# Shadylukin/Neumann

Measured on AMD Instinct MI355X. Metric: queries/sec, brute-force SIMILAR TOP-K (recall@K = 1.0 vs CPU oracle), higher is better.
Workload: dtype f32

## Files before the change

### neumann_amd/csrc/nmn_api.hip

```cpp
#include <algorithm>
#include <atomic>
#include <chrono>
#include <thread>
#include <cmath>
#include <cstdio>
#include <cstdlib>
#include <cstring>
#include <mutex>
#include <new>
#include <string>
#include <unordered_map>
#include <vector>

#include "nmn_index.h"

using namespace nmn;

namespace nmn {
float synth_value_host(uint64_t seed, uint64_t row, uint32_t col);
}

static thread_local std::string g_last_error;

static nmn_status fail_hip(hipError_t e, const char* what) {
// ... 950 lines not shown
        if (qmasks_host && !use_mfma) {
            const bool mark = w->timed && qa == 0 && !nested;
            if (mark && (st = hist_mark(0)) != NMN_OK) return st;
            for (uint32_t i = 0; i < nqc; i++) {
                st = search_enqueue(idx, w, queries_dev + (size_t)(qa + i) * idx->dim, 1, k, metric, qmasks_host[qa + i],
                                    out_rows + (size_t)(qa + i) * k, out_scores + (size_t)(qa + i) * k, out_counts + qa + i,
                                    stream, nullptr, nullptr, short_chain, true);
                if (st != NMN_OK) return st;
            }
            if (mark && (st = hist_mark(1)) != NMN_OK) return st;
            continue;
        }
        w->last_elem_bytes = use_i8 ? 1u : use_half ? 2u : 4u;
        static const bool two_planes = env_set("NMN_I8_TWO_PLANES");
        const bool pipelined = idx->sweep_seq != 0 && idx->sweep_stream != stream;
        const bool one_plane = use_i8 && use_mfma && !two_planes && metric == NMN_METRIC_COSINE && k <= 128u && (nqc > 64u || !pipelined) &&
                               scan_mfma_i8_one_plane_supported((int)metric) && idx->q8_calls >= idx->one_plane_off_until;
        if (one_plane) idx->one_plane_recent = true;
        const bool f32_retry = (use_half || use_i8) && !use_mfma && n_rows >= (1u << 18) && !short_chain;
        static const bool no_run_bound = env_set("NMN_NO_RUN_BOUND");
        static const bool wgs_pinned = getenv("NMN_MFMA_WGS") != nullptr;
        const bool run_bound = use_mfma && !no_run_bound && !no_sample() && !mask_dev && !qmasks_dev && k <= 256u && nqc <= 64u && !wgs_pinned &&
                               idx->ld <= 1536u &&
                               n_tiles >= 1024u * kSampleStep && n_tiles / kSampleStep >= 4u * k;
        const uint32_t run_S = run_bound ? k : 0u;
        HIP_TRY(launch_qprep(queries_dev + (size_t)qa * idx->dim, nqc, idx->dim, idx->ld, (int)metric,
                             idx->max_norm_bits, w->qpad, w->qinfo, w->qstate,
                             use_i8 ? (1 | 2 | 4 | (use_mfma ? (one_plane ? 16 : 0) : 8)) : ((use_mfma ? 1 : 0) | ((use_half || mfma_f32) ? 2 : 0)), stream,
                             use_i8 ? idx->q8_err_bits : (use_half || (mfma_f32 && idx->half && idx->half_rows >= n_rows)) ? idx->half_err_bits : nullptr,
                             use_i8 ? w->qi8 : nullptr,
                             (use_i8 && !use_mfma) ? idx->q8_l2_hint : nullptr, f32_retry ? w->qinfo_f32 : nullptr,
                             run_bound ? w->run_slots : nullptr, run_S, run_bound ? w->run_bound : nullptr));
        if (n_rows > 0) {
            ScanParams sp{};
            sp.corpus = idx->corpus;
            sp.corpus_half = use_half ? idx->half : nullptr;
            sp.corpus_i8 = use_i8 ? idx->q8 : nullptr;
            sp.i8_one_plane = one_plane ? 1u : 0u;
            sp.i8_scale = idx->q8_scale;
            sp.i8_vv = idx->q8_vv;
            sp.i8_cos = idx->q8_cos;
            sp.qi8 = w->qi8;
            sp.norms = idx->norms;
            sp.inv_norms = idx->inv_norms;
            sp.qpad = w->qpad;
            sp.qinfo = w->qinfo;
            sp.mask = mask_dev;
// ... 11 lines not shown
            static const uint32_t wave_target = [] {
                const char* e = getenv("NMN_SCAN_WAVES");
                long v = e ? atol(e) : (long)kMaxScanWaves;
                return (uint32_t)std::min<long>(std::max<long>(v, 256), (long)kMaxScanWaves);
            }();
            sp.tiles_per_wave = std::max<uint32_t>(1, (n_tiles + wave_target - 1) / wave_target);
            static const bool waves_pinned = getenv("NMN_SCAN_WAVES") != nullptr;
            static const uint32_t small_waves = [] {
                const char* e = getenv("NMN_SCAN_WAVES_SMALL");
                const long v = e ? atol(e) : 768;
                return v <= 0 ? 0u : (uint32_t)std::min<long>(std::max<long>(v, 256), (long)kMaxScanWaves);
            }();
            {
                const uint64_t sweep_bytes = (uint64_t)n_rows * idx->ld * w->last_elem_bytes;
                if (!waves_pinned && small_waves && !use_mfma && !mask_dev && sweep_bytes >= (128ull << 20) && sweep_bytes < (2ull << 30))
                    sp.tiles_per_wave = std::max<uint32_t>(1, (n_tiles + small_waves - 1) / small_waves);
            }
            static const uint32_t mfma_wgs = [] {
                const char* e = getenv("NMN_MFMA_WGS");
                long v = e ? atol(e) : 1024;
                return (uint32_t)std::min<long>(std::max<long>(v, 64), (long)kMaxScanWaves);
            }();
            if (use_mfma) sp.tiles_per_wave = std::max<uint32_t>(1, (n_tiles + mfma_wgs - 1) / mfma_wgs);
            auto launch_batch_sweep = [&](const ScanParams& x) -> hipError_t { return launch_scan_mfma(x, stream); };
            static const bool no_ring = getenv("NMN_NO_RING") != nullptr;
            const bool use_ring = !no_ring && !use_mfma && !use_i8 && !use_half && nqc == 1 && !mask_dev && !qmasks_dev && n_tiles >= 4096u &&
                                  metric != NMN_METRIC_SPARSE_COSINE_F64 && scan_ring_supported(idx->ld, idx->dim, (int)metric);
            static const uint32_t ring_wgs = [] {
                const char* e = getenv("NMN_RING_WGS");
                long v = e ? atol(e) : (long)kMaxScanWaves;
                return (uint32_t)std::min<long>(std::max<long>(v, 64), (long)kMaxScanWaves);
            }();
            if (use_ring) sp.tiles_per_wave = std::max<uint32_t>(1, (n_tiles + ring_wgs - 1) / ring_wgs);
            ring_set_grid(sp, use_ring ? w->ring_ctr : nullptr);
            sp.metric = (int)metric;
            sp.strided = (!use_mfma && mask_dev) ? 1u : 0u;
            static const bool no_walk = getenv("NMN_NO_WALK") != nullptr;
            sp.walk = (sp.strided && !no_walk) ? 1u : 0u;
            sp.tile_step = 1;
            sp.skip_key = nullptr;
            static const uint32_t sample_step = [] {
                const char* e = getenv("NMN_SAMPLE_STEP");
                const long v = e ? atol(e) : 0;
                return (v == 64 || v == 128 || v == 256) ? (uint32_t)v : kSampleStep;
            }();
            static const bool sample_behind = getenv("NMN_SAMPLE_AHEAD_OF_CHAIN") == nullptr;
// ... 13 lines not shown
                ss.n_tiles = n_sample;
                ss.tiles_per_wave = std::max<uint32_t>(1, (n_sample + 255) / 256);
                ss.tmax = w->tsample;
                ss.tmax_stride = w->n_sample_cap;
                static const bool reread_env = getenv("NMN_SAMPLE_REREAD") != nullptr;
                const bool reread = reread_env || use_i8;
                if (!reread) {
                    ss.tmax_main = w->tmax;
                    ss.tmax_main_stride = w->tmax_stride;
                }
                HIP_TRY(launch_batch_sweep(ss));
                HIP_TRY(launch_sample_bound(w->tsample, w->n_sample_cap, n_sample, w->qinfo, nqc, k, w->skip_key, stream));
                sp.skip_key = w->skip_key;
                sp.skip_sampled = reread ? 0u : sample_step;
                return NMN_OK;
            };
            if (sample && !sample_behind) {
                st = sampling_pass();
                if (st != NMN_OK) return st;
            }
            static const bool no_chain = getenv("NMN_NO_SWEEP_CHAIN") != nullptr;
            const bool chain = !no_chain && (uint64_t)n_rows * idx->ld * w->last_elem_bytes >= (2ull << 30);
            if (sp.ring_wgs) HIP_TRY(hipMemsetAsync(w->wmax, 0, (size_t)((n_tiles + sp.tiles_per_wave - 1) / sp.tiles_per_wave) * sizeof(uint32_t), stream));
            if (chain && idx->sweep_seq && idx->sweep_stream != stream)
                HIP_TRY(hipStreamWaitEvent(stream, idx->sweep_ev[(idx->sweep_seq - 1) & 3u], 0));
            if (w->timed && qa == 0 && !nested) {
                hipEvent_t& h = w->hist[2 * (w->hist_head % Workspace::kTimingHistory)];
                if (!h) HIP_TRY(hipEventCreate(&h));
                HIP_TRY(hipEventRecord(h, stream));
            }
            if (sample && sample_behind) {
                st = sampling_pass();
                if (st != NMN_OK) return st;
            }
            static const bool no_refine = getenv("NMN_NO_REFINE") != nullptr;
            const uint32_t mfma_blocks = use_mfma ? (n_tiles + sp.tiles_per_wave - 1) / sp.tiles_per_wave : 0;
            static const uint32_t n_cu = [] {
                int dev = 0, n = 256;
                if (hipGetDevice(&dev) != hipSuccess || hipDeviceGetAttribute(&n, hipDeviceAttributeMultiprocessorCount, dev) != hipSuccess || n <= 0) n = 256;
                return (uint32_t)n;
            }();
            const uint32_t first_blocks = mfma_blocks >= 3u * n_cu ? (n_cu & ~7u) : 0u;
            static const uint32_t refine_min_nq = [] {
                const char* e = getenv("NMN_REFINE_MIN_NQ");
                return e ? (uint32_t)atol(e) : 65u;
            }();
// ... 1152 lines not shown
```

### neumann_amd/csrc/nmn_internal.h

```cpp
#pragma once
#include <hip/hip_runtime.h>
#include <stdint.h>

#include "../../include/neumann_gpu.h"

namespace nmn {

constexpr int kMetricNegL2 = 16;
constexpr int kMetricNegL2Sq = 17;

constexpr uint32_t kTileRows = 64;
constexpr uint32_t kDefaultCandCap = 4096;
constexpr uint32_t kMaxScanWaves = 4096;
constexpr uint32_t kKeyMasked = 0u;
constexpr uint32_t kKeyNaN = 1u;
constexpr uint32_t kScoreSentinelBits = 0xFFFFFFFFu;

struct QInfo {
    float qmag;
    float margin_abs;
    float margin_rel;
    float pad;
    float qscale;
    float qq8;
// ... 99 lines not shown
    uint64_t n_rows;
    uint32_t nql;
    uint32_t tile_step;
    uint32_t fold_ny;
    const uint32_t* skip_key;
    uint32_t* tmax_main;
    uint64_t tmax_main_stride;
    uint32_t skip_sampled;
    uint32_t ld;
    uint32_t n_tiles;
    uint32_t nq;
    uint32_t tiles_per_wave;
    uint32_t strided;
    uint32_t walk;
    uint32_t bx_base, bx_count;
    uint32_t* run_slots;
    uint32_t* run_bound;
    uint32_t run_S;
    uint32_t i8_one_plane;
    uint32_t ring_wgs;
    uint32_t ring_tail;
    uint32_t ring_grid;
    uint32_t* ring_ctr;
    uint32_t run_dbg;
    int metric;
};
hipError_t launch_scan(const ScanParams& p, hipStream_t s);
bool scan_ring_supported(uint32_t ld, uint32_t dim, int metric);
hipError_t launch_scan_ring(const ScanParams& p, hipStream_t s);
hipError_t launch_half_rows(const float* corpus, float* half, uint32_t ld, uint64_t row0, uint64_t n, const float* norms,
                            float* row_err2_scratch, uint32_t* err_bits, hipStream_t s);
bool scan_half_supported(uint32_t ld, int metric);
bool scan_i8_supported(uint32_t ld, uint32_t dim, int metric);
hipError_t launch_scan_i8(const ScanParams& p, hipStream_t s);
hipError_t launch_q8_rows(const float* corpus, int8_t* q8, float* scale, float* vv, float* cosf, uint32_t ld, uint64_t row0, uint64_t n, const float* norms,
                          float* row_err2_scratch, uint32_t* err_bits, hipStream_t s);
bool ingest_supported(uint32_t ld, uint32_t dim);
bool exact_rows_supported(uint32_t ld, uint32_t dim, int metric);
hipError_t launch_exact_rows(const float* corpus, const float* norms, uint32_t ld, uint64_t n_rows, const float* qpad, const QInfo* qinfo,
                             const QState* qstate, int flagged, const uint64_t* mask, const uint64_t* const* qmasks, uint32_t* scores,
                             uint32_t nql, uint32_t nq, int metric, hipStream_t s);
hipError_t launch_ingest(const float* corpus, uint32_t ld, uint64_t row0, uint64_t n, float* norms, float* inv_norms,
                         uint32_t* max_norm_bits, float* half, uint32_t* err_bits, hipStream_t s);
bool ingest_q8_supported(uint32_t ld, uint32_t dim);
hipError_t launch_ingest_q8(const float* corpus, uint32_t ld, uint64_t row0, uint64_t n, float* norms, float* inv_norms, uint32_t* max_norm_bits,
                            int8_t* q8, float* scale, float* vv, float* cosf, uint32_t* err_bits, hipStream_t s);
hipError_t launch_read_probe(const float* corpus, uint64_t n_rows, uint32_t ld, float* sink, hipStream_t s);
hipError_t launch_ring_probe(const float* corpus, uint64_t n_rows, uint32_t ld, uint32_t tiles_per_wg, uint32_t* ctr, hipStream_t s);
void ring_set_grid(ScanParams& p, uint32_t* ctr);
bool scan_mfma_supported(uint32_t ld, uint32_t dim, int metric);
hipError_t launch_scan_mfma(const ScanParams& p, hipStream_t s);
hipError_t launch_scan_mfma_f32(const ScanParams& p, hipStream_t s);
bool scan_mfma_i8_supported(uint32_t ld, uint32_t dim, int metric);
bool scan_mfma_i8_one_plane_supported(int metric);
hipError_t launch_scan_mfma_i8_one(const ScanParams& p, hipStream_t s);

struct SelectParams {
    const uint32_t* scores;
    const uint32_t* tmax;
    const uint32_t* wmax;
    uint64_t tmax_stride;
    uint64_t wmax_stride;
    uint32_t n_waves;
    uint32_t tiles_per_wave;
    uint32_t strided;
    const QInfo* qinfo;
    QState* qstate;
    uint32_t* cand_rows;
    uint64_t n_rows;
    uint32_t nql;
    uint32_t n_tiles;
    uint32_t nq;
// ... 177 lines not shown
```

### neumann_amd/csrc/nmn_scan_mfma.hip

```cpp
#include "nmn_scan_mfma_kernel.h"

namespace nmn {

template <int KC, int KS, int QG, int METRIC, int WAVES = 4>
static hipError_t launch_kc(const ScanParams& p, hipStream_t s) {
    return (p.mask || p.qmasks) ? launch_one_mfma<KC, KS, QG, METRIC, true, WAVES>(p, s)
                                : launch_one_mfma<KC, KS, QG, METRIC, false, WAVES>(p, s);
}

template <int METRIC>
static hipError_t launch_metric(const ScanParams& p, hipStream_t s) {
    static const bool waves8 = [] {
        const char* e = getenv("NMN_MFMA_WAVES");
        return e ? atoi(e) == 8 : false;
    }();
    if (waves8) {
        if (p.nq > 64) {
            switch (p.ld / kStageK) {
                case 6: return launch_kc<3, 2, 8, METRIC, 8>(p, s);
                default: break;
            }
        } else {
            switch (p.ld / kStageK) {
                case 6: return launch_kc<3, 2, 4, METRIC, 8>(p, s);
// ... 72 lines not shown
        case 5: return launch_kc_i8<5, 1, METRIC>(p, s);
        case 6: return launch_kc_i8<3, 2, METRIC>(p, s);
        case 8: return launch_kc_i8<4, 2, METRIC, 2>(p, s);
        case 12: return launch_kc_i8<6, 2, METRIC, 2>(p, s);
        default: return hipErrorInvalidValue;
    }
}
bool scan_mfma_i8_supported(uint32_t ld, uint32_t dim, int metric) {
    if (!(metric == NMN_METRIC_COSINE || metric == NMN_METRIC_DOT_PRODUCT || metric == NMN_METRIC_EUCLIDEAN || metric == kMetricNegL2))
        return false;
    if (ld == 3072u && (metric == NMN_METRIC_EUCLIDEAN || metric == kMetricNegL2)) return false;
    return dim <= ld && ld % 256u == 0 && ld >= 256u && (ld <= 1536u || ld == 2048u || ld == 3072u);
}

bool scan_mfma_supported(uint32_t ld, uint32_t dim, int metric) {
    if (!(metric == NMN_METRIC_COSINE || metric == NMN_METRIC_DOT_PRODUCT || metric == NMN_METRIC_EUCLIDEAN ||
          metric == kMetricNegL2) ||
        dim > ld || ld % kStageK != 0)
        return false;
    const uint32_t kc = ld / kStageK;
    return (kc >= 1 && kc <= 6) || kc == 8 || kc == 10 || kc == 12 || kc == 16 || kc == 24 || kc == 32;
}

hipError_t launch_scan_mfma(const ScanParams& p, hipStream_t s) {
    if (!p.corpus_i8 && !p.corpus_half) return launch_scan_mfma_f32(p, s);
    if (p.corpus_i8 && p.i8_one_plane) return launch_scan_mfma_i8_one(p, s);
    if (p.corpus_i8) {
        switch (p.metric) {
            case NMN_METRIC_COSINE: return launch_metric_i8<NMN_METRIC_COSINE>(p, s);
            case NMN_METRIC_EUCLIDEAN: return launch_metric_i8<NMN_METRIC_EUCLIDEAN>(p, s);
            case kMetricNegL2: return launch_metric_i8<kMetricNegL2>(p, s);
            default: return launch_metric_i8<NMN_METRIC_DOT_PRODUCT>(p, s);
        }
    }
    switch (p.metric) {
        case NMN_METRIC_COSINE: return launch_metric<NMN_METRIC_COSINE>(p, s);
        case NMN_METRIC_EUCLIDEAN: return launch_metric<NMN_METRIC_EUCLIDEAN>(p, s);
        case kMetricNegL2: return launch_metric<kMetricNegL2>(p, s);
        default: return launch_metric<NMN_METRIC_DOT_PRODUCT>(p, s);
    }
}

}
```

### neumann_amd/csrc/nmn_scan_mfma_kernel.h

```cpp
#pragma once
#include <algorithm>
#include <cstdlib>
#include <type_traits>

#include "nmn_internal.h"

namespace nmn {

typedef float f4 __attribute__((ext_vector_type(4)));
typedef short s8 __attribute__((ext_vector_type(8)));
typedef uint32_t u4 __attribute__((ext_vector_type(4)));

#ifndef NMN_MFMA_BATCH
#define NMN_MFMA_BATCH 8
#endif
constexpr int kStageK = 128;
#ifndef NMN_MFMA_RING_KB
#define NMN_MFMA_RING_KB 128
#endif
#ifndef NMN_MFMA_OCC
#define NMN_MFMA_OCC 1
#endif
#ifdef NMN_MFMA_NO_FENCES
#define NMN_MFMA_FENCE() do { } while (0)
#else
#define NMN_MFMA_FENCE() __builtin_amdgcn_sched_barrier(0)
#endif
constexpr int kRingBytes = NMN_MFMA_RING_KB * 1024;

typedef float f2 __attribute__((ext_vector_type(2)));
typedef __bf16 bf2 __attribute__((ext_vector_type(2)));

__device__ __forceinline__ uint32_t cvt_pk_bf16(float lo, float hi) {
    const f2 v = {lo, hi};
    return __builtin_bit_cast(uint32_t, __builtin_convertvector(v, bf2));
}

__device__ __forceinline__ s8 to_bf16x8(const f4& a, const f4& b) {
    u4 h;
    h[0] = cvt_pk_bf16(a.x, a.y);
    h[1] = cvt_pk_bf16(a.z, a.w);
    h[2] = cvt_pk_bf16(b.x, b.y);
    h[3] = cvt_pk_bf16(b.z, b.w);
    return __builtin_bit_cast(s8, h);
}

constexpr int kNormSlots = 16;

template <int AUX, int PIECES>
__device__ __forceinline__ void stage_dma(const char* stage_base, const uint32_t (&loff)[PIECES], float* buf,
                                          uint32_t wave) {
#pragma unroll
    for (int pp = 0; pp < PIECES; pp++) {
        const char* src = stage_base + loff[pp];
        __builtin_amdgcn_global_load_lds((const __attribute__((address_space(1))) void*)src,
                                         (__attribute__((address_space(3))) void*)(buf + (wave * PIECES + (uint32_t)pp) * 256u),
                                         16, 0, AUX);
    }
}

template <int AUX, int PIECES>
__device__ __forceinline__ void stage_dma_piece(const char* stage_base, const uint32_t (&loff)[PIECES], float* buf, uint32_t wave,
                                                int pp) {
    __builtin_amdgcn_global_load_lds((const __attribute__((address_space(1))) void*)(stage_base + loff[pp]),
                                     (__attribute__((address_space(3))) void*)(buf + (wave * PIECES + (uint32_t)pp) * 256u), 16, 0, AUX);
}

__device__ __forceinline__ void norms_dma(const float* __restrict__ norms, uint64_t tile, float* nbuf, uint32_t lane) {
// ... 32 lines not shown
    const float d2 = __builtin_fmaxf(__builtin_fmaf(-2.0f, dot, qq8 + vv), 0.0f);
    const float d = __builtin_amdgcn_sqrtf(d2);
    return NEG ? -d : __builtin_amdgcn_rcpf(1.0f + d);
}

template <int KS, int QG, int WAVES, bool I8>
__host__ __device__ constexpr uint32_t kRunLdsBase() {
    return (uint32_t)(kRingBytes + kNormSlots * 64 * 4 + (QG * 2 == WAVES ? QG * 64 * 4 * 16 : 0) +
                      WAVES * (QG * 2 == WAVES ? 1 : QG / WAVES) * 16 * 16 +
#ifdef NMN_MFMA_PACK
                      (I8 ? kNormSlots * 64 * 4 + WAVES * (16 * 64 + 16) * 4 : 0));
#else
                      (I8 ? kNormSlots * 64 * 4 : 0));
#endif
}
constexpr int kRunVals = 1024;
template <int QG>
__host__ __device__ constexpr uint32_t kRunLdsRing() { return (uint32_t)(kNormSlots * QG * 16 * 4); }
template <int QG, int WAVES>
__host__ __device__ constexpr uint32_t kRunLdsBytes() {
    return kRunLdsRing<QG>() + (uint32_t)(QG * 16 * (int)sizeof(QInfo) + WAVES * kRunVals * 4);
}

template <int KC, int KS, int QG, int METRIC, bool MASKED, int AUX, int WAVES, bool I8 = false, bool F32 = false, bool ONE = false>
__global__ void __launch_bounds__(WAVES * 64, NMN_MFMA_OCC) scan_mfma_kernel(ScanParams p) {
    static_assert(!(I8 && F32), "one streamed matrix");
    static_assert(!ONE || I8, "one query plane: the 8-bit form only");
    constexpr int kStageElems = 128 * KS;
    constexpr int kStageBytes = kTileRows * kStageElems * 2;
    constexpr int kRowPitch = kStageElems / 2;
    constexpr int kRing = kRingBytes / kStageBytes;
    constexpr int kPieces = 16 * KS / WAVES;
    constexpr uint32_t LR = 16 * KS;
    constexpr bool kL2 = METRIC == NMN_METRIC_EUCLIDEAN || METRIC == kMetricNegL2;
    constexpr bool kNeedNorms = I8 || METRIC == NMN_METRIC_COSINE || kL2;
    constexpr bool kScaled = METRIC == NMN_METRIC_COSINE || (I8 && METRIC == NMN_METRIC_DOT_PRODUCT);
    extern __shared__ __attribute__((aligned(16))) float lds[];
    float* nrm = lds + kRingBytes / 4;
    float* const nrm2 = nrm + kNormSlots * 64 + (QG * 2 == WAVES ? QG * 64 * 16 : 0) + WAVES * (QG * 2 == WAVES ? 1 : QG / WAVES) * 16 * 4;
#ifdef NMN_MFMA_PACK
    constexpr bool kPack = I8;
#else
    constexpr bool kPack = false;
#endif
    float* const pack_lds = nrm2 + kNormSlots * 64;
    constexpr uint32_t kQ = (uint32_t)QG * 16u;
    uint32_t* const bnd = reinterpret_cast<uint32_t*>(lds) + (kRunLdsBase<KS, QG, WAVES, I8>() >> 2);
    QInfo* const qmrg = reinterpret_cast<QInfo*>(bnd + kNormSlots * kQ);
    uint32_t* const slotb = reinterpret_cast<uint32_t*>(qmrg + kQ);
    const uint32_t run_S = p.run_S;
    const uint32_t lane = threadIdx.x & 63u;
    const uint32_t wave = __builtin_amdgcn_readfirstlane(threadIdx.x >> 6);
    const uint32_t g = lane >> 4, n = lane & 15u;
    const uint32_t ld = p.ld;
    const uint32_t row_bytes = I8 ? ld : F32 ? ld * 4u : ld * 2u;
    uint32_t bx = blockIdx.x, by = blockIdx.y;
    if (p.fold_ny > 1) {
        const uint32_t span = 8u * p.fold_ny, grp_ = blockIdx.x / span, r_ = blockIdx.x % span;
        by = r_ / 8u;
        bx = grp_ * 8u + (r_ % 8u);
    }
    if (p.bx_count && bx >= p.bx_count) return;
    bx += p.bx_base;
    const uint32_t q0 = by * (uint32_t)(QG * 16);
    constexpr bool kHalfK = QG * 2 == WAVES;
    static_assert(kHalfK || QG % WAVES == 0, "query groups: one (or more) per wave, or one per wave PAIR");
    const uint32_t grp = kHalfK ? (wave % (uint32_t)QG) : wave;
    const uint32_t kh = kHalfK ? (wave / (uint32_t)QG) : 0u;

    constexpr int kStageSteps = F32 ? 2 * KS : 4 * KS;
    constexpr int kSteps = kHalfK ? kStageSteps / 2 : kStageSteps;
    static_assert(kSteps >= 1, "K-halves need two k-steps per stage");
    constexpr int kBK = KC * kSteps;
    constexpr int kBG = kHalfK ? 1 : QG / WAVES;
    s8 bhi[kBK][kBG];
    s8 blo[(I8 && !ONE) ? kBK : 1][kBG];
#pragma unroll
    for (int qg = 0; qg < kBG; qg++) {
        const uint32_t qq = q0 + ((uint32_t)qg * (uint32_t)WAVES + grp) * 16u + n;
        const bool ok = qq < p.nq;
        const float* qv = p.qpad + (size_t)(ok ? qq : q0) * ld;
        if constexpr (I8) {
            const char* qb = reinterpret_cast<const char*>(p.qi8) + (size_t)(ok ? qq : q0) * 2u * ld;
#pragma unroll
            for (int kc = 0; kc < kBK; kc++) {
                const uint32_t k0b = ((uint32_t)(kc / kSteps) * (4u * KS) + kh * (uint32_t)kSteps + (uint32_t)(kc % kSteps)) * 64u + g * 16u;
// ... 36 lines not shown
        skip_h[h] = (q_ok_h[h] && p.skip_key) ? p.skip_key[qn_h[h]] : kKeyNaN;
        wmax_h[h] = kKeyMasked;
    }

    if (run_S) {
        for (uint32_t i = threadIdx.x; i < kQ; i += (uint32_t)WAVES * 64u)
            qmrg[i] = p.qinfo[min(q0 + i, p.nq - 1u)];
        __syncthreads();
    }
#ifndef NMN_RUN_PICK
#define NMN_RUN_PICK 4
#endif
    constexpr uint32_t kPick = NMN_RUN_PICK;
    auto bound_dma = [&](uint32_t rel) __attribute__((always_inline)) {
        if (rel % kPick) return;
#pragma unroll
        for (uint32_t h = 0; h < kQ; h += 64u)
            __builtin_amdgcn_global_load_lds((const __attribute__((address_space(1))) void*)(p.run_bound + q0 + h + lane),
                                             (__attribute__((address_space(3))) void*)(bnd + ((rel / kPick) % kNormSlots) * kQ + h), 4, 0, 16);
    };
    uint32_t pend_q = 0xFFFFFFFFu;
    const uint32_t tstep = p.tile_step;
    const bool sampling = tstep > 1;
    const uint32_t t0 = bx * p.tiles_per_wave;
    if (t0 >= p.n_tiles) return;
    const uint32_t t1 = min(t0 + p.tiles_per_wave, p.n_tiles);
    const uint32_t S = sampling ? 0u : p.skip_sampled;
    auto walked_below = [&](uint32_t t) -> uint32_t { return S ? t - (t + S - 1u) / S : t; };
    auto tile_of = [&](uint32_t j) -> uint32_t { return S ? j + j / (S - 1u) + 1u : j; };
    const uint32_t j0 = walked_below(t0), j1 = walked_below(t1);
    const uint32_t n_stage = (j1 - j0) * KC;

    uint32_t loff[kPieces];
#pragma unroll
    for (int pp = 0; pp < kPieces; pp++) {
        const uint32_t r = (64u / LR) * (wave * kPieces + (uint32_t)pp) + lane / LR;
        loff[pp] = r * row_bytes + (((lane % LR) ^ (r & 15u)) * 16u);
    }
    const char* const mirror = I8 ? reinterpret_cast<const char*>(p.corpus_i8)
                                  : F32 ? reinterpret_cast<const char*>(p.corpus) : reinterpret_cast<const char*>(p.corpus_half);
    const float* const norm_src = I8 ? (METRIC == NMN_METRIC_COSINE ? p.i8_cos : p.i8_scale)
                                     : (METRIC == NMN_METRIC_COSINE ? p.inv_norms : p.norms);
    auto stage_src = [&](uint32_t tile_, uint32_t kc_) -> const char* {
        return mirror + (uint64_t)tile_ * tstep * kTileRows * row_bytes + (uint64_t)kc_ * (kStageElems * 2u);
    };

#pragma unroll
    for (uint32_t s0 = 0; s0 < kRing; s0++) {
        if (s0 < n_stage) {
            if (run_S && !(p.run_dbg & 8u) && wave == 0 && s0 % KC == 0) bound_dma(s0 / KC);
            if (kNeedNorms && wave == 0 && s0 % KC == 0)
            {
                norms_dma(norm_src, (uint64_t)tile_of(j0 + s0 / KC) * tstep, nrm + ((s0 / KC) % kNormSlots) * 64u, lane);
                if constexpr (I8 && kL2) norms_dma(p.i8_vv, (uint64_t)tile_of(j0 + s0 / KC) * tstep, nrm2 + ((s0 / KC) % kNormSlots) * 64u, lane);
            }
            if (s0 < kRing - 1)
                stage_dma<AUX, kPieces>(stage_src(tile_of(j0 + s0 / KC), s0 % KC), loff, lds + (s0 % kRing) * (kStageBytes / 4), wave);
        } else if (s0 < kRing - 1) {
            const uint32_t zero[kPieces] = {};
            stage_dma<AUX, kPieces>(mirror, zero, lds + (s0 % kRing) * (kStageBytes / 4), wave);
        }
    }

    uint32_t off[kSteps];
#pragma unroll
    for (int ks = 0; ks < kSteps; ks++)
        off[ks] = F32 ? n * kRowPitch + ((((kh * (uint32_t)kSteps + (uint32_t)ks) * 8u + g * 2u) ^ n) * 4u)
                      : n * kRowPitch + ((((kh * (uint32_t)kSteps + (uint32_t)ks) * 4u + g) ^ n) * 4u);
// ... 35 lines not shown
            if (q_ok && g == 0) p.tmax[(uint64_t)qn * p.tmax_stride + ftile] = tkey;
#else
            {
                const uint32_t slot = ftile & 3u;
                uint32_t* mine = tk_pend + (((uint32_t)wave * (uint32_t)kHalves + (uint32_t)H) * 16u + n) * 4u;
                if (g == 0) mine[slot] = tkey;
                if (slot == 3u || flast) {
                    const uint32_t g0 = ftile & ~3u, first = max((S && g0 % S == 0u) ? g0 + 1u : g0, t0);
                    if (q_ok && g == 0) {
                        uint32_t* dst = p.tmax + (uint64_t)qn * p.tmax_stride + g0;
                        const u4 v = *reinterpret_cast<const u4*>(mine);
                        if (first == g0 && slot == 3u && (p.tmax_stride & 3ull) == 0ull) {
                            *reinterpret_cast<u4*>(dst) = v;
                        } else {
                            if (first <= g0 + 0u) dst[0] = v[0];
                            if (first <= g0 + 1u && slot >= 1u) dst[1] = v[1];
                            if (first <= g0 + 2u && slot >= 2u) dst[2] = v[2];
                            if (first <= g0 + 3u && slot >= 3u) dst[3] = v[3];
                        }
                    }
                }
            }
#endif
            if (run_S && !(p.run_dbg & 2u) && q_ok && g == 0 && tkey > wmax_h[H] && !sampling) p.run_slots[(size_t)qn * (uint32_t)kRunVals + bx] = tkey;
            wmax_h[H] = max(wmax_h[H], tkey);
            const bool finish_sampled = sampling && p.tmax_main != nullptr;
            if (finish_sampled && q_ok && g == 0) p.tmax_main[(uint64_t)qn * p.tmax_main_stride + rtile] = tkey;
#ifdef NMN_MFMA_NO_SCORE_WRITES
            return false;
#else
            const bool wr_ = q_ok && (!sampling || finish_sampled) && tkey != kKeyMasked && tkey >= skip;
            return wr_;
#endif
        };
        constexpr bool kLazy = METRIC == NMN_METRIC_COSINE || METRIC == NMN_METRIC_DOT_PRODUCT;
        auto l2_of = [&](float acc_v, float vn_v, float vv_v) __attribute__((always_inline)) -> float {
            if constexpr (I8) return l2_score_i8<METRIC == kMetricNegL2>(qq, vv_v, acc_v * (inv_q * vn_v));
            else return l2_score<METRIC == kMetricNegL2>(qq, vn_v, acc_v);
        };
        if (mword == ~0ull) {
            float m = -__builtin_inff();
            u4 bits[4];
#pragma unroll
            for (int rb = 0; rb < 4; rb++) {
                f4 sc = fin[rb];
                if constexpr (kScaled) {
                    sc = sc * npre[rb];
// ... 36 lines not shown
#pragma unroll
                        for (int rb = 0; rb < 4; rb++) *reinterpret_cast<u4*>(stage + rank * 64u + (uint32_t)rb * 16u + g * 4u) = words(rb);
                        if (g == 0) qsel[rank] = qn;
                    }
                    asm volatile("" ::: "memory");
                    const uint32_t nw = (uint32_t)__builtin_popcount(qm);
                    for (uint32_t b = 0; b < nw; b += 4u) {
                        const uint32_t slot = b + (lane >> 4), piece = lane & 15u;
                        if (slot < nw) {
                            const u4 v = *reinterpret_cast<const u4*>(stage + slot * 64u + piece * 4u);
                            *reinterpret_cast<u4*>(p.scores + score_at(r0 + piece * 4u, qsel[slot], p.nql)) = v;
                        }
                    }
                    asm volatile("" ::: "memory");
                }
            } else if (wr) {
#pragma unroll
                for (int rb = 0; rb < 4; rb++)
                    *reinterpret_cast<u4*>(p.scores + score_at(r0 + (uint32_t)rb * 16u + g * 4u, qn, p.nql)) = words(rb);
            }
        } else {
            uint32_t tkey = kKeyMasked;
            u4 bits[4];
#pragma unroll
            for (int rb = 0; rb < 4; rb++) {
                const uint32_t rr = (uint32_t)rb * 16u + g * 4u;
                f4 vn = {1.f, 1.f, 1.f, 1.f}, vv = {0.f, 0.f, 0.f, 0.f};
                if constexpr (kNeedNorms) vn = npre[rb];
                if constexpr (I8 && kL2) vv = *reinterpret_cast<const f4*>(nslot2 + rr);
#pragma unroll
                for (int e = 0; e < 4; e++) {
                    const bool valid = ((mword >> (rr + (uint32_t)e)) & 1ull) != 0;
                    float sc = fin[rb][e];
                    if constexpr (kScaled) sc = (sc * vn[e]) * inv_q;
                    if constexpr (kL2) sc = l2_of(sc, vn[e], vv[e]);
                    bits[rb][e] = valid ? f2u(sc) : kScoreSentinelBits;
                    if (valid) tkey = max(tkey, score_to_key(sc));
                }
            }
            if (publish(tkey)) {
#pragma unroll
                for (int rb = 0; rb < 4; rb++)
                    *reinterpret_cast<u4*>(p.scores + score_at(r0 + (uint32_t)rb * 16u + g * 4u, qn, p.nql)) = bits[rb];
            }
        }
    };
    auto finish_tile = [&](const f4 (&facc)[4][kAccGroups], uint32_t ftile, uint32_t frel, bool flast, const f4 (&npre)[4],
                           const uint32_t (&skp)[kHalves]) __attribute__((always_inline)) {
#ifdef NMN_MFMA_NO_EPILOGUE
// ... 16 lines not shown
        const uint32_t tile = tile_of(j);
        f4 acc[4][kAccGroups];
        f4 npre[4] = {{1.f, 1.f, 1.f, 1.f}, {1.f, 1.f, 1.f, 1.f}, {1.f, 1.f, 1.f, 1.f}, {1.f, 1.f, 1.f, 1.f}};
        uint32_t skp[kHalves];
#pragma unroll
        for (int h = 0; h < kHalves; h++) skp[h] = kKeyNaN;
        v4i ach[I8 ? 4 : 1][kAccGroups], acl[I8 ? 4 : 1][kAccGroups];
#pragma unroll
        for (int rb = 0; rb < 4; rb++)
#pragma unroll
            for (int qg = 0; qg < kAccGroups; qg++) {
                acc[rb][qg] = (f4){0.f, 0.f, 0.f, 0.f};
                if constexpr (I8) {
                    ach[rb][qg] = (v4i){0, 0, 0, 0};
                    acl[rb][qg] = (v4i){0, 0, 0, 0};
                }
            }
#pragma unroll
        for (int kc = 0; kc < KC; kc++, sidx++) {
            const float* buf = lds + (sidx % kRing) * (kStageBytes / 4);
            wait_vm_imm<(kRing - 2) * kPieces>();
            __builtin_amdgcn_s_barrier();
            asm volatile("" ::: "memory");
            const uint32_t ns = sidx + (kRing - 1);
            const bool issue = ns < n_stage;
            const uint32_t nt = tile_of(j0 + ns / KC), nkc = ns % KC;
            const char* const nsrc = issue ? stage_src(nt, nkc) : mirror;
            const uint32_t lmask = issue ? 0xFFFFFFFFu : 0u;
            float* const nbuf = lds + (ns % kRing) * (kStageBytes / 4);
            constexpr int kKsPerBatch = F32 ? 1 : (kBK * kBG * (I8 ? 8 : 4) >= (I8 ? 192 : 256)) ? 1 : 2;
            static_assert(kSteps % kKsPerBatch == 0, "batches tile the stage");
            constexpr int kNB = kSteps / kKsPerBatch;
            s8 a[F32 ? 1 : kSteps][4];
            u4 raw[F32 ? kSteps : 1][4][2];
            auto read_batch = [&](int b) __attribute__((always_inline)) {
#pragma unroll
                for (int ks = b * kKsPerBatch; ks < (b + 1) * kKsPerBatch; ks++)
#pragma unroll
                    for (int rb = 0; rb < 4; rb++) {
                        if constexpr (F32) {
                            const uint32_t o0 = off[ks], o1 = off[ks] ^ 4u;
                            raw[ks][rb][0] = *reinterpret_cast<const u4*>(buf + rb * 16 * kRowPitch + o0);
                            raw[ks][rb][1] = *reinterpret_cast<const u4*>(buf + rb * 16 * kRowPitch + o1);
                        } else {
                            a[ks][rb] = __builtin_bit_cast(s8, *reinterpret_cast<const u4*>(buf + rb * 16 * kRowPitch + off[ks]));
                        }
                    }
            };
// ... 90 lines not shown
                for (int rb = 0; rb < 4; rb++)
                    *reinterpret_cast<f4*>(xch + ((grp * 64u + lane) * 4u + (uint32_t)rb) * 4u) = acc[rb][0];
            }
            asm volatile("s_waitcnt lgkmcnt(0)" ::: "memory");
            __builtin_amdgcn_s_barrier();
            asm volatile("" ::: "memory");
            if (kh == 0) {
#pragma unroll
                for (int rb = 0; rb < 4; rb++)
                    acc[rb][0] += *reinterpret_cast<const f4*>(xch + ((grp * 64u + lane) * 4u + (uint32_t)rb) * 4u);
            }
            asm volatile("s_waitcnt lgkmcnt(0)" ::: "memory");
            finish_tile(acc, tile, j - j0, j + 1u == j1, npre, skp);
        } else {
            finish_tile(acc, tile, j - j0, j + 1u == j1, npre, skp);
        }
        if (run_S && !(p.run_dbg & 4u)) {
#ifndef NMN_RUN_REFRESH
#define NMN_RUN_REFRESH 64
#endif
            constexpr uint32_t kRefresh = NMN_RUN_REFRESH;
            constexpr uint32_t kDelay = (uint32_t)((kRing - 2 + KC - 1) / KC);
            static_assert(kDelay >= 1 && kDelay < kRefresh, "refresh timing");
            const uint32_t rel = j - j0, phase = bx % kRefresh;
            if ((rel % kRefresh) == (phase + kDelay) % kRefresh && pend_q != 0xFFFFFFFFu) {
                wait_vm_imm<(kRing - 2) * kPieces>();
                uint32_t v[kRunVals / 64];
#pragma unroll
                for (int i = 0; i < kRunVals / 256; i++) {
                    const u4 x = *reinterpret_cast<const u4*>(slotb + wave * (uint32_t)kRunVals + (uint32_t)i * 256u + lane * 4u);
                    v[4 * i + 0] = x[0]; v[4 * i + 1] = x[1]; v[4 * i + 2] = x[2]; v[4 * i + 3] = x[3];
                }
                uint32_t pre = 0;
                for (int bit = 31; bit >= 10; bit--) {
                    const uint32_t c = pre | (1u << bit);
                    uint32_t cnt = 0;
#pragma unroll
                    for (int i = 0; i < kRunVals / 64; i++) cnt += (uint32_t)__builtin_popcountll(__ballot(v[i] >= c));
                    if (cnt >= run_S) pre = c;
                }
                if (pre > kKeyNaN && lane == 0) atomicMax(p.run_bound + pend_q, margin_key(pre, qmrg[pend_q - q0]));
            }
            if ((rel % kRefresh) == phase) {
                const uint32_t turn = ((rel / kRefresh) + bx) % (16u * (uint32_t)kBG);
                const uint32_t qq = q0 + ((turn / 16u) * (uint32_t)WAVES + grp) * 16u + (turn % 16u);
                pend_q = (kh == 0 && qq < p.nq) ? qq : 0xFFFFFFFFu;
                if (pend_q != 0xFFFFFFFFu) {
#pragma unroll
                    for (int i = 0; i < kRunVals / 256; i++)
                        __builtin_amdgcn_global_load_lds((const __attribute__((address_space(1))) void*)(p.run_slots + (size_t)pend_q * (uint32_t)kRunVals + (uint32_t)i * 256u + lane * 4u),
                                                         (__attribute__((address_space(3))) void*)(slotb + wave * (uint32_t)kRunVals + (uint32_t)i * 256u), 16, 0, 16);
                }
            }
        }
    }
    wait_vm_imm<0>();
    if (sampling) return;
#pragma unroll
    for (int h = 0; h < kHalves; h++)
        if (q_ok_h[h] && g == 0) {
            if (S)
                for (uint32_t ts = ((t0 + S - 1u) / S) * S; ts < t1; ts += S)
                    wmax_h[h] = max(wmax_h[h], p.tmax[(uint64_t)qn_h[h] * p.tmax_stride + ts]);
            p.wmax[(size_t)qn_h[h] * p.wmax_stride + bx] = wmax_h[h];
        }
}

template <int KC, int KS, int QG, int METRIC, bool MASKED, int WAVES, bool I8 = false, bool F32 = false, bool ONE = false>
static hipError_t launch_one_mfma(const ScanParams& p, hipStream_t s) {
    const uint32_t blocks_all = (p.n_tiles + p.tiles_per_wave - 1) / p.tiles_per_wave;
    if (p.bx_base >= blocks_all) return hipSuccess;
    const uint32_t blocks = p.bx_count ? std::min(p.bx_count, blocks_all - p.bx_base) : blocks_all - p.bx_base;
    const uint32_t ny = (p.nq + QG * 16 - 1) / (QG * 16);
    ScanParams pf = p;
    pf.bx_count = blocks;
    dim3 grid(blocks, ny);
    static const bool no_fold = getenv("NMN_MFMA_NO_FOLD") != nullptr;
    if (ny > 1 && !no_fold) {
        pf.fold_ny = ny;
        grid = dim3(((blocks + 7u) / 8u) * 8u * ny, 1);
    }
    const size_t lds = (size_t)kRunLdsBase<KS, QG, WAVES, I8>() + (p.run_S ? (size_t)kRunLdsBytes<QG, WAVES>() : (size_t)kRunLdsRing<QG>());
    if (lds > 160u * 1024u) return hipErrorInvalidValue;
    if (p.skip_sampled && (p.skip_sampled < 4u || (p.skip_sampled & 3u))) return hipErrorInvalidValue;
    if (p.run_S && (p.run_S > 256u || blocks_all > (uint32_t)kRunVals || p.tile_step > 1u || (p.skip_sampled && !(p.run_dbg & 1u)))) return hipErrorInvalidValue;
#ifndef NMN_MFMA_AUX
#define NMN_MFMA_AUX 2
#endif
    auto kern = scan_mfma_kernel<KC, KS, QG, METRIC, MASKED, NMN_MFMA_AUX, WAVES, I8, F32, ONE>;
    hipError_t e = hipFuncSetAttribute(reinterpret_cast<const void*>(kern), hipFuncAttributeMaxDynamicSharedMemorySize,
                                       (int)lds);
    if (e != hipSuccess) return e;
    hipLaunchKernelGGL(kern, grid, dim3(WAVES * 64), lds, s, pf);
    return hipGetLastError();
}

}
```

Baseline: 225.7.

## Add persistent one-launch MFMA sweep with atomic-ticket work stealing over split tile chunks

Under the run-bound path, the MFMA scan kernel now launches one workgroup per CU. Each workgroup pulls chunk tickets from an atomic counter, and each 1024-way tile group is divided into several parts, with finer parts for the tail groups. Partial per-group maxima are merged with atomicMax into run_slots and wmax, which are cleared beforehand with a memset. The goal is to remove tail imbalance and wave quantization across CUs. The cost is atomics, extra barriers per chunk, a memset, and a counter that the last workgroup must reset.

New measurement: 225.2, median of 2. No clear change (-0.2%).

```diff
diff --git a/neumann_amd/csrc/nmn_api.hip b/neumann_amd/csrc/nmn_api.hip
--- a/neumann_amd/csrc/nmn_api.hip
+++ b/neumann_amd/csrc/nmn_api.hip
@@ -996,7 +996,8 @@
         static const bool wgs_pinned = getenv("NMN_MFMA_WGS") != nullptr;
         const bool run_bound = use_mfma && !no_run_bound && !no_sample() && !mask_dev && !qmasks_dev && k <= 256u && nqc <= 64u && !wgs_pinned &&
                                idx->ld <= 1536u &&
-                               n_tiles >= 1024u * kSampleStep && n_tiles / kSampleStep >= 4u * k;
+                               n_tiles >= 1024u * kSampleStep && n_tiles / kSampleStep >= 4u * k &&
+                               scan_mfma_run_bound_fits(idx->ld, use_i8 ? 1u : use_half ? 2u : 4u, nqc);
         const uint32_t run_S = run_bound ? k : 0u;
         HIP_TRY(launch_qprep(queries_dev + (size_t)qa * idx->dim, nqc, idx->dim, idx->ld, (int)metric,
                              idx->max_norm_bits, w->qpad, w->qinfo, w->qstate,
@@ -1054,6 +1055,7 @@
                 return (uint32_t)std::min<long>(std::max<long>(v, 64), (long)kMaxScanWaves);
             }();
             if (use_mfma) sp.tiles_per_wave = std::max<uint32_t>(1, (n_tiles + mfma_wgs - 1) / mfma_wgs);
+            if (use_mfma) mfma_set_grid(sp, run_bound ? w->ring_ctr : nullptr);
             auto launch_batch_sweep = [&](const ScanParams& x) -> hipError_t { return launch_scan_mfma(x, stream); };
             static const bool no_ring = getenv("NMN_NO_RING") != nullptr;
             const bool use_ring = !no_ring && !use_mfma && !use_i8 && !use_half && nqc == 1 && !mask_dev && !qmasks_dev && n_tiles >= 4096u &&
@@ -1113,6 +1115,8 @@
             static const bool no_chain = getenv("NMN_NO_SWEEP_CHAIN") != nullptr;
             const bool chain = !no_chain && (uint64_t)n_rows * idx->ld * w->last_elem_bytes >= (2ull << 30);
             if (sp.ring_wgs) HIP_TRY(hipMemsetAsync(w->wmax, 0, (size_t)((n_tiles + sp.tiles_per_wave - 1) / sp.tiles_per_wave) * sizeof(uint32_t), stream));
+            if (use_mfma && sp.even_chunks)
+                HIP_TRY(hipMemset2DAsync(w->wmax, (size_t)kMaxScanWaves * sizeof(uint32_t), 0, (size_t)((n_tiles + sp.tiles_per_wave - 1) / sp.tiles_per_wave) * sizeof(uint32_t), nqc, stream));
             if (chain && idx->sweep_seq && idx->sweep_stream != stream)
                 HIP_TRY(hipStreamWaitEvent(stream, idx->sweep_ev[(idx->sweep_seq - 1) & 3u], 0));
             if (w->timed && qa == 0 && !nested) {
diff --git a/neumann_amd/csrc/nmn_internal.h b/neumann_amd/csrc/nmn_internal.h
--- a/neumann_amd/csrc/nmn_internal.h
+++ b/neumann_amd/csrc/nmn_internal.h
@@ -145,6 +145,8 @@
     uint32_t ring_tail;
     uint32_t ring_grid;
     uint32_t* ring_ctr;
+    uint32_t even_chunks, even_main_groups, even_main_parts, even_tail_parts, even_align, even_grid;
+    uint32_t* even_ctr;
     uint32_t run_dbg;
     int metric;
 };
@@ -171,6 +173,8 @@
 hipError_t launch_read_probe(const float* corpus, uint64_t n_rows, uint32_t ld, float* sink, hipStream_t s);
 hipError_t launch_ring_probe(const float* corpus, uint64_t n_rows, uint32_t ld, uint32_t tiles_per_wg, uint32_t* ctr, hipStream_t s);
 void ring_set_grid(ScanParams& p, uint32_t* ctr);
+void mfma_set_grid(ScanParams& p, uint32_t* ctr);
+bool scan_mfma_run_bound_fits(uint32_t ld, uint32_t elem_bytes, uint32_t nq);
 bool scan_mfma_supported(uint32_t ld, uint32_t dim, int metric);
 hipError_t launch_scan_mfma(const ScanParams& p, hipStream_t s);
 hipError_t launch_scan_mfma_f32(const ScanParams& p, hipStream_t s);
diff --git a/neumann_amd/csrc/nmn_scan_mfma.hip b/neumann_amd/csrc/nmn_scan_mfma.hip
--- a/neumann_amd/csrc/nmn_scan_mfma.hip
+++ b/neumann_amd/csrc/nmn_scan_mfma.hip
@@ -118,6 +118,31 @@
     return (kc >= 1 && kc <= 6) || kc == 8 || kc == 10 || kc == 12 || kc == 16 || kc == 24 || kc == 32;
 }
 
+bool scan_mfma_run_bound_fits(uint32_t ld, uint32_t elem_bytes, uint32_t nq) {
+    if (nq > 64u || ld > 1536u) return false;
+    const uint32_t lds = (elem_bytes == 1u ? kRunLdsBase<1, 4, 4, true>() : kRunLdsBase<1, 4, 4, false>()) + kRunLdsBytes<4, 4>() + kEvenLdsBytes;
+    return lds <= 160u * 1024u;
+}
+
+void mfma_set_grid(ScanParams& p, uint32_t* ctr) {
+    struct Knobs {
+        bool on;
+        uint32_t main, tail, align, cus;
+    };
+    static const Knobs k = []() -> Knobs {
+        int dev = 0, n = 256;
+        if (hipGetDevice(&dev) != hipSuccess || hipDeviceGetAttribute(&n, hipDeviceAttributeMultiprocessorCount, dev) != hipSuccess || n <= 0) n = 256;
+        auto knob = [](const char* name, long def, long lo, long hi) {
+            const char* e = getenv(name);
+            return (uint32_t)std::min<long>(std::max<long>(e ? atol(e) : def, lo), hi);
+        };
+        return {getenv("NMN_NO_MFMA_EVEN") == nullptr, knob("NMN_MFMA_MAIN", 6, 1, 1024), knob("NMN_MFMA_TAIL", 8, 0, 4096), knob("NMN_MFMA_ALIGN", 4, 1, 64),
+                (uint32_t)n};
+    }();
+    p.even_chunks = 0;
+    if (ctr && k.on) mfma_even_split(p, k.main, k.tail, k.align, k.cus, ctr);
+}
+
 hipError_t launch_scan_mfma(const ScanParams& p, hipStream_t s) {
     if (!p.corpus_i8 && !p.corpus_half) return launch_scan_mfma_f32(p, s);
     if (p.corpus_i8 && p.i8_one_plane) return launch_scan_mfma_i8_one(p, s);
diff --git a/neumann_amd/csrc/nmn_scan_mfma_kernel.h b/neumann_amd/csrc/nmn_scan_mfma_kernel.h
--- a/neumann_amd/csrc/nmn_scan_mfma_kernel.h
+++ b/neumann_amd/csrc/nmn_scan_mfma_kernel.h
@@ -44,6 +44,13 @@
     h[3] = cvt_pk_bf16(b.z, b.w);
     return __builtin_bit_cast(s8, h);
 }
+
+#ifdef NMN_MFMA_WG_CLOCK
+__device__ unsigned long long* nmn_mfma_clk;
+#define NMN_MFMA_CLK(i, v) do { if (threadIdx.x == 0) nmn_mfma_clk[(uint64_t)blockIdx.x * 5u + (i)] = (v); } while (0)
+#else
+#define NMN_MFMA_CLK(i, v) do { } while (0)
+#endif
 
 constexpr int kNormSlots = 16;
 
@@ -122,7 +129,9 @@
     return kRunLdsRing<QG>() + (uint32_t)(QG * 16 * (int)sizeof(QInfo) + WAVES * kRunVals * 4);
 }
 
-template <int KC, int KS, int QG, int METRIC, bool MASKED, int AUX, int WAVES, bool I8 = false, bool F32 = false, bool ONE = false>
+constexpr uint32_t kEvenLdsBytes = 16;
+
+template <int KC, int KS, int QG, int METRIC, bool MASKED, int AUX, int WAVES, bool I8 = false, bool F32 = false, bool ONE = false, bool EVEN = false>
 __global__ void __launch_bounds__(WAVES * 64, NMN_MFMA_OCC) scan_mfma_kernel(ScanParams p) {
     static_assert(!(I8 && F32), "one streamed matrix");
     static_assert(!ONE || I8, "one query plane: the 8-bit form only");
@@ -148,12 +157,15 @@
     uint32_t* const bnd = reinterpret_cast<uint32_t*>(lds) + (kRunLdsBase<KS, QG, WAVES, I8>() >> 2);
     QInfo* const qmrg = reinterpret_cast<QInfo*>(bnd + kNormSlots * kQ);
     uint32_t* const slotb = reinterpret_cast<uint32_t*>(qmrg + kQ);
+    uint32_t* const ticket = slotb + (uint32_t)WAVES * (uint32_t)kRunVals;
     const uint32_t run_S = p.run_S;
     const uint32_t lane = threadIdx.x & 63u;
     const uint32_t wave = __builtin_amdgcn_readfirstlane(threadIdx.x >> 6);
     const uint32_t g = lane >> 4, n = lane & 15u;
     const uint32_t ld = p.ld;
     const uint32_t row_bytes = I8 ? ld : F32 ? ld * 4u : ld * 2u;
+    NMN_MFMA_CLK(0, wall_clock64());
+    NMN_MFMA_CLK(4, __smid());
     uint32_t bx = blockIdx.x, by = blockIdx.y;
     if (p.fold_ny > 1) {
         const uint32_t span = 8u * p.fold_ny, grp_ = blockIdx.x / span, r_ = blockIdx.x % span;
@@ -162,6 +174,10 @@
     }
     if (p.bx_count && bx >= p.bx_count) return;
     bx += p.bx_base;
+    const uint32_t even = EVEN ? p.even_chunks : 0u;
+    const uint32_t wg = even ? blockIdx.x : bx;
+    uint32_t next_ticket = 0;
+    if (even && threadIdx.x == 0) next_ticket = atomicAdd(p.even_ctr, 1u);
     const uint32_t q0 = by * (uint32_t)(QG * 16);
     constexpr bool kHalfK = QG * 2 == WAVES;
     static_assert(kHalfK || QG % WAVES == 0, "query groups: one (or more) per wave, or one per wave PAIR");
@@ -244,14 +260,9 @@
     uint32_t pend_q = 0xFFFFFFFFu;
     const uint32_t tstep = p.tile_step;
     const bool sampling = tstep > 1;
-    const uint32_t t0 = bx * p.tiles_per_wave;
-    if (t0 >= p.n_tiles) return;
-    const uint32_t t1 = min(t0 + p.tiles_per_wave, p.n_tiles);
     const uint32_t S = sampling ? 0u : p.skip_sampled;
     auto walked_below = [&](uint32_t t) -> uint32_t { return S ? t - (t + S - 1u) / S : t; };
     auto tile_of = [&](uint32_t j) -> uint32_t { return S ? j + j / (S - 1u) + 1u : j; };
-    const uint32_t j0 = walked_below(t0), j1 = walked_below(t1);
-    const uint32_t n_stage = (j1 - j0) * KC;
 
     uint32_t loff[kPieces];
 #pragma unroll
@@ -266,6 +277,42 @@
     auto stage_src = [&](uint32_t tile_, uint32_t kc_) -> const char* {
         return mirror + (uint64_t)tile_ * tstep * kTileRows * row_bytes + (uint64_t)kc_ * (kStageElems * 2u);
     };
+
+    uint32_t wrel = 0;
+    for (uint32_t round = 0;; round++) {
+    uint32_t t0 = bx * p.tiles_per_wave, t1 = t0 + p.tiles_per_wave;
+    bool split = false;
+    if (even) {
+        __syncthreads();
+        if (threadIdx.x == 0) *ticket = next_ticket;
+        __syncthreads();
+        const uint32_t c = __builtin_amdgcn_readfirstlane(*ticket);
+        if (c >= even) break;
+        if (threadIdx.x == 0) next_ticket = atomicAdd(p.even_ctr, 1u);
+        const uint32_t cm = p.even_main_groups * p.even_main_parts;
+        const uint32_t parts = c < cm ? p.even_main_parts : p.even_tail_parts;
+        const uint32_t cc = c < cm ? c : c - cm;
+        bx = (c < cm ? 0u : p.even_main_groups) + cc / parts;
+        const uint32_t part = cc % parts;
+        const uint32_t g0 = bx * p.tiles_per_wave, g1 = min(g0 + p.tiles_per_wave, p.n_tiles);
+        auto border = [&](uint32_t i) -> uint32_t {
+            if (i == 0u) return g0;
+            if (i >= parts) return g1;
+            const uint32_t b = g0 + (uint32_t)((uint64_t)(g1 - g0) * i / parts);
+            return max(b - b % p.even_align, g0);
+        };
+        t0 = border(part);
+        t1 = border(part + 1u);
+        if (t1 <= t0) continue;
+        split = parts > 1u;
+#pragma unroll
+        for (int h = 0; h < kHalves; h++) wmax_h[h] = kKeyMasked;
+    } else {
+        if (round || t0 >= p.n_tiles) break;
+        t1 = min(t1, p.n_tiles);
+    }
+    const uint32_t j0 = walked_below(t0), j1 = walked_below(t1);
+    const uint32_t n_stage = (j1 - j0) * KC;
 
 #pragma unroll
     for (uint32_t s0 = 0; s0 < kRing; s0++) {
@@ -347,7 +394,11 @@
                 }
             }
 #endif
-            if (run_S && !(p.run_dbg & 2u) && q_ok && g == 0 && tkey > wmax_h[H] && !sampling) p.run_slots[(size_t)qn * (uint32_t)kRunVals + bx] = tkey;
+            if (run_S && !(p.run_dbg & 2u) && q_ok && g == 0 && tkey > wmax_h[H] && !sampling && (!split || tkey >= skip)) {
+                uint32_t* const word = p.run_slots + (size_t)qn * (uint32_t)kRunVals + bx;
+                if (split) atomicMax(word, tkey);
+                else *word = tkey;
+            }
             wmax_h[H] = max(wmax_h[H], tkey);
             const bool finish_sampled = sampling && p.tmax_main != nullptr;
             if (finish_sampled && q_ok && g == 0) p.tmax_main[(uint64_t)qn * p.tmax_main_stride + rtile] = tkey;
@@ -430,9 +481,11 @@
         } else {
             uint32_t tkey = kKeyMasked;
             u4 bits[4];
+            uint32_t g_here = g;
+            asm volatile("" : "+v"(g_here));
 #pragma unroll
             for (int rb = 0; rb < 4; rb++) {
-                const uint32_t rr = (uint32_t)rb * 16u + g * 4u;
+                const uint32_t rr = (uint32_t)rb * 16u + g_here * 4u;
                 f4 vn = {1.f, 1.f, 1.f, 1.f}, vv = {0.f, 0.f, 0.f, 0.f};
                 if constexpr (kNeedNorms) vn = npre[rb];
                 if constexpr (I8 && kL2) vv = *reinterpret_cast<const f4*>(nslot2 + rr);
@@ -495,8 +548,14 @@
             wait_vm_imm<(kRing - 2) * kPieces>();
             __builtin_amdgcn_s_barrier();
             asm volatile("" ::: "memory");
+#ifdef NMN_MFMA_WG_CLOCK
+            if (kc == 0 && j == j0 && wrel == 0) NMN_MFMA_CLK(1, wall_clock64());
+#endif
             const uint32_t ns = sidx + (kRing - 1);
             const bool issue = ns < n_stage;
+#ifdef NMN_MFMA_WG_CLOCK
+            if (ns == n_stage || (sidx == 0 && ns > n_stage)) NMN_MFMA_CLK(2, wall_clock64());
+#endif
             const uint32_t nt = tile_of(j0 + ns / KC), nkc = ns % KC;
             const char* const nsrc = issue ? stage_src(nt, nkc) : mirror;
             const uint32_t lmask = issue ? 0xFFFFFFFFu : 0u;
@@ -633,7 +692,7 @@
             constexpr uint32_t kRefresh = NMN_RUN_REFRESH;
             constexpr uint32_t kDelay = (uint32_t)((kRing - 2 + KC - 1) / KC);
             static_assert(kDelay >= 1 && kDelay < kRefresh, "refresh timing");
-            const uint32_t rel = j - j0, phase = bx % kRefresh;
+            const uint32_t rel = wrel + (j - j0), phase = wg % kRefresh;
             if ((rel % kRefresh) == (phase + kDelay) % kRefresh && pend_q != 0xFFFFFFFFu) {
                 wait_vm_imm<(kRing - 2) * kPieces>();
                 uint32_t v[kRunVals / 64];
@@ -653,7 +712,7 @@
                 if (pre > kKeyNaN && lane == 0) atomicMax(p.run_bound + pend_q, margin_key(pre, qmrg[pend_q - q0]));
             }
             if ((rel % kRefresh) == phase) {
-                const uint32_t turn = ((rel / kRefresh) + bx) % (16u * (uint32_t)kBG);
+                const uint32_t turn = ((rel / kRefresh) + wg) % (16u * (uint32_t)kBG);
                 const uint32_t qq = q0 + ((turn / 16u) * (uint32_t)WAVES + grp) * 16u + (turn % 16u);
                 pend_q = (kh == 0 && qq < p.nq) ? qq : 0xFFFFFFFFu;
                 if (pend_q != 0xFFFFFFFFu) {
@@ -666,6 +725,7 @@
         }
     }
     wait_vm_imm<0>();
+    wrel += j1 - j0;
     if (sampling) return;
 #pragma unroll
     for (int h = 0; h < kHalves; h++)
@@ -673,8 +733,35 @@
             if (S)
                 for (uint32_t ts = ((t0 + S - 1u) / S) * S; ts < t1; ts += S)
                     wmax_h[h] = max(wmax_h[h], p.tmax[(uint64_t)qn_h[h] * p.tmax_stride + ts]);
-            p.wmax[(size_t)qn_h[h] * p.wmax_stride + bx] = wmax_h[h];
-        }
+            uint32_t* const word = p.wmax + (size_t)qn_h[h] * p.wmax_stride + bx;
+            if (split) atomicMax(word, wmax_h[h]);
+            else *word = wmax_h[h];
+        }
+    if constexpr (!EVEN) break;
+    }
+    if (even && threadIdx.x == 0 && atomicAdd(p.even_ctr + 1, 1u) == gridDim.x - 1u) {
+        p.even_ctr[0] = 0u;
+        p.even_ctr[1] = 0u;
+    }
+    NMN_MFMA_CLK(3, wall_clock64());
+}
+
+inline void mfma_even_split(ScanParams& p, uint32_t main, uint32_t tail, uint32_t align, uint32_t cus, uint32_t* ctr) {
+    p.even_chunks = 0;
+    p.even_ctr = ctr;
+    if (!ctr || !main || !cus || !align || p.n_tiles == 0 || p.tiles_per_wave == 0) return;
+    const uint32_t tpw = p.tiles_per_wave, groups = (p.n_tiles + tpw - 1) / tpw;
+    const double share = (double)p.n_tiles / ((double)cus * (4.0 * main + tail));
+    auto parts_of = [&](double chunk_tiles) {
+        return (uint32_t)std::min<double>(std::max<double>((double)tpw / std::max(chunk_tiles, 1.0) + 0.5, 1.0), (double)tpw);
+    };
+    p.even_main_parts = parts_of(4.0 * share);
+    p.even_tail_parts = std::max(parts_of(share), p.even_main_parts);
+    const uint32_t tail_groups = (uint32_t)((double)groups * tail / (4.0 * main + tail) + 0.5);
+    p.even_main_groups = groups - std::min(tail_groups, groups);
+    p.even_align = align;
+    p.even_grid = cus;
+    p.even_chunks = p.even_main_groups * p.even_main_parts + (groups - p.even_main_groups) * p.even_tail_parts;
 }
 
 template <int KC, int KS, int QG, int METRIC, bool MASKED, int WAVES, bool I8 = false, bool F32 = false, bool ONE = false>
@@ -686,19 +773,33 @@
     ScanParams pf = p;
     pf.bx_count = blocks;
     dim3 grid(blocks, ny);
+    if (p.even_chunks && !(p.run_S && ny == 1 && !MASKED && QG == 4 && WAVES == 4 && p.tile_step == 1 && !p.skip_sampled && !p.bx_base && !p.bx_count && p.even_ctr &&
+                           p.even_grid && p.even_main_parts && p.even_tail_parts && p.even_align))
+        pf.even_chunks = 0;
+    if (pf.even_chunks) {
+        pf.bx_count = 0;
+        grid = dim3(pf.even_grid, 1);
+    }
     static const bool no_fold = getenv("NMN_MFMA_NO_FOLD") != nullptr;
     if (ny > 1 && !no_fold) {
         pf.fold_ny = ny;
         grid = dim3(((blocks + 7u) / 8u) * 8u * ny, 1);
     }
-    const size_t lds = (size_t)kRunLdsBase<KS, QG, WAVES, I8>() + (p.run_S ? (size_t)kRunLdsBytes<QG, WAVES>() : (size_t)kRunLdsRing<QG>());
+    static_assert(!(QG == 4 && WAVES == 4 && NMN_MFMA_RING_KB == 128) || kRunLdsBase<KS, QG, WAVES, I8>() + kRunLdsBytes<QG, WAVES>() + kEvenLdsBytes <= 160u * 1024u,
+                  "the one-launch sweep's LDS request exceeds 160 KiB");
+    const size_t lds = (size_t)kRunLdsBase<KS, QG, WAVES, I8>() + (p.run_S ? (size_t)kRunLdsBytes<QG, WAVES>() : (size_t)kRunLdsRing<QG>()) +
+                       (pf.even_chunks ? (size_t)kEvenLdsBytes : 0u);
     if (lds > 160u * 1024u) return hipErrorInvalidValue;
     if (p.skip_sampled && (p.skip_sampled < 4u || (p.skip_sampled & 3u))) return hipErrorInvalidValue;
     if (p.run_S && (p.run_S > 256u || blocks_all > (uint32_t)kRunVals || p.tile_step > 1u || (p.skip_sampled && !(p.run_dbg & 1u)))) return hipErrorInvalidValue;
 #ifndef NMN_MFMA_AUX
 #define NMN_MFMA_AUX 2
 #endif
+    constexpr bool kCanEven = !MASKED && QG == 4 && WAVES == 4;
+    if (pf.even_chunks && !kCanEven) return hipErrorInvalidValue;
     auto kern = scan_mfma_kernel<KC, KS, QG, METRIC, MASKED, NMN_MFMA_AUX, WAVES, I8, F32, ONE>;
+    if constexpr (kCanEven)
+        if (pf.even_chunks) kern = scan_mfma_kernel<KC, KS, QG, METRIC, MASKED, NMN_MFMA_AUX, WAVES, I8, F32, ONE, true>;
     hipError_t e = hipFuncSetAttribute(reinterpret_cast<const void*>(kern), hipFuncAttributeMaxDynamicSharedMemorySize,
                                        (int)lds);
     if (e != hipSuccess) return e;
```
